# NuclearnAI/nuclear-sim

Measured on AMD Instinct MI355X. Metric: plant-env-steps/s, higher is better.
Workload: dtype f64

## Files before the change

nuclear_sim_amd/csrc/npd_step4.h:

```cpp
#ifndef NPD_STEP4_H
#define NPD_STEP4_H

#define NPD4_THREADS 256
#ifndef NPD4_NO_ELIDE
#define NPD4_ST_STORE(T, stype, s, old, inst) NPD_ST_STORE_ELIDE(T, stype, s, old, inst)
#else
#define NPD4_ST_STORE(T, stype, s, old, inst) NPD_ST_STORE(T, stype, s, inst)
#endif
#define NPD4_SLOTS 142
#ifdef NPB_STAMPS
#define NPD4_STAMP(k) do { if (lane == 0 && npb_stamp_buf) npb_stamp_buf[((size_t)blockIdx.x * 4 + wave) * 32 + (k)] = __builtin_readcyclecounter(); } while (0)
#else
#define NPD4_STAMP(k)
#endif
enum { FL_CHAIN = 0, FL_FWFLOW = 1, FL_PRIM = 2, FL_FWCTL = 3, FL_PUMP = 4 , FL_SG = 8 , FL_PASSA = 11, FL_UNIT = 12 ,
       FL_POST = 15 , FL_VERDICT = 18, FL_TAIL = 19, FL_CONDP = 20, FL_LUBE = 21, FL_CHAINDONE = 22, FL_COUNT = 23 };
#define NPD4_FLAGP(n) ((volatile int *)&xch[Y_FLAGS * NPB_WAVE + 2 * (n)])
#define NPD4_FLAG_SET(n, v) do { asm volatile("" ::: "memory"); *NPD4_FLAGP(n) = (v); asm volatile("" ::: "memory"); } while (0)
#ifndef NPD4_POLL_SLEEP
#define NPD4_POLL_SLEEP 1
#endif
#define NPD4_FLAG_WAIT(n, v) do { while (__builtin_amdgcn_readfirstlane(*NPD4_FLAGP(n)) < (v)) __builtin_amdgcn_s_sleep(NPD4_POLL_SLEEP); asm volatile("" ::: "memory"); } while (0)
#define NPD4_UNIT_WAIT(u) do { if ((u) < 12) NPD4_FLAG_WAIT(FL_UNIT + (u) % 2, (u) / 2 + 1); else NPD4_FLAG_WAIT(FL_UNIT + 2, (u) - 11); } while (0)

enum {
  Y_EXTF = 0, Y_TIN = 5, Y_STEAM = 6, Y_CHRES = 7,
  Y_CFLOW = 0, Y_CIN = 3, Y_COUT = 6, Y_LDF = 9, Y_FWTEMP = 10, Y_NPREV = 11, Y_FPP = 12, Y_MAXLVL = 13, Y_RUNCOUNT = 14, Y_FWFLOW = 15,
  Y_PRIM = 16,
  Y_TIME = 22, Y_FLAGS = 23, Y_MAINT_TAB = 24,
  Y_PUMP = 25,
  Y_SAT = 25, Y_HG = 40, Y_TRATIO = 55, Y_HGEXT = 69,
  Y_OBS = 25, Y_INFO = 48,
  Y_SG = 77,
  Y_TOUT = 77,
  Y_PSELF = 95, Y_PEXT = 109, Y_PIN = 114,
  Y_TAIL = 95,
  Y_LOADING = 116, Y_STRESS = 130, Y_CWT = 140, Y_CONDP = 141
};
static_assert(Y_PUMP + 4 * X_PUMP_N <= Y_SG && Y_HGEXT + 5 <= Y_SG && Y_INFO + NPB_OBS_PAD <= Y_SG && Y_OBS + NPB_OBS_PAD <= Y_INFO && Y_SG + 18 <= Y_PSELF &&
              Y_TOUT + 14 <= Y_PSELF && Y_TAIL + 21 <= Y_LOADING && Y_PIN < Y_LOADING && Y_LOADING + 14 <= Y_STRESS && Y_STRESS + 8 <= Y_CWT && Y_CHRES + 7 <= Y_FWFLOW &&
              Y_CONDP < NPD4_SLOTS && 2 * FL_COUNT <= NPB_WAVE && NPD_MH_N + 8 <= NPB_WAVE, "exchange slot plan");

template <int K0, int K1>
__device__ __forceinline__ void npd4_store_turb_range(const npd_stage_t &st, const npb_turb_t &t, const npb_turb_t &t_old) {
  const double *d = reinterpret_cast<const double *>(&t), *od = reinterpret_cast<const double *>(&t_old);
#pragma unroll
  for (int k = K0; k < K1; k++) {
    if ((NPD_ELIDE_TURB_F >> k) & 1) {
      if (__builtin_amdgcn_ballot_w64(npd_real_bits(d[k]) != npd_real_bits(od[k])) != 0) *NPD_RP(NPD_SEC_COL(TURB, 0) + k) = (npd_real_t)d[k];
    } else {
      *NPD_RP(NPD_SEC_COL(TURB, 0) + k) = (npd_real_t)d[k];
    }
  }
}

#ifndef NPD4_UNITS_FIRST
#define NPD4_UNITS_FIRST 1
#endif
template <int R>
__device__ __forceinline__ void npd4_stage_preload(const npd_stage_t &st, npd_tstg_old_t &old) {
#define NPD4_OLD(member, k) (old.v[NPD_TSTG_SLOT(member, k)] = (double)NPD2_TSTG(member, k))
#pragma unroll
  for (int j = 0; j < 5; j++) {
    const int k = R + 3 * j;
    if (k >= 14) continue;
    NPD4_OLD(stage_efficiency_degradation, k); NPD4_OLD(stage_deposit_thickness, k);
    NPD4_OLD(stage_blade_wear_factor, k); NPD4_OLD(blade_temperatures, k);
    if (k < 8) NPD4_OLD(rotor_temperatures, k);
    if (k < 6) NPD4_OLD(casing_temperatures, k);
  }
#undef NPD4_OLD
}
template <int R>
__device__ __forceinline__ void npd4_stage_post(const npd_stage_t &st, const npd_tstg_old_t &old, double *xch, int lane, double tdt) {
  NPD4_FLAG_WAIT(FL_VERDICT, 1);
  const int base = (__builtin_amdgcn_readfirstlane(*NPD4_FLAGP(FL_VERDICT)) == 2) ? 100 : 0;
#pragma unroll
  for (int j = 0; j < 5; j++) {
    const int k = R + 3 * j;
    if (k >= 14) continue;
    NPD4_FLAG_WAIT(FL_CHAIN, base + k + 1);
    const double stress = npd_stage_post<NPD_SM>(st, k, old, XR(Y_LOADING + k), XR(Y_TOUT + k), tdt).stress;
    if (k < 8) XW(Y_STRESS + (k < 8 ? k : 0), stress);
  }
  NPD4_FLAG_SET(FL_POST + R, 1);
}
template <int U0, int STEP, int COUNT, int WHOSE>
__device__ __forceinline__ void npd4_pass_b_units(double *xch, int lane) {
#pragma unroll
  for (int j = 0; j < COUNT; j++) {
    const int u = U0 + STEP * j;
    if (u == 0) {
      NPD4_FLAG_WAIT(FL_PASSA, 1);
      const double sat = npd_tsat_antoine(XR(Y_PIN));
      XW(Y_SAT + 0, sat); XW(Y_HG + 0, npd_hg_from_tsat(sat));
    } else {
      const int k = u - 1;
      NPD4_FLAG_WAIT(FL_PASSA, k + 2);
      const double pk = XR(Y_PSELF + (k >= 0 ? k : 0)), pkm = (k == 0) ? XR(Y_PIN) : XR(Y_PSELF + (k > 0 ? k - 1 : 0));
      const double sat = npd_tsat_antoine(pk);
      XW(Y_SAT + u, sat); XW(Y_HG + u, npd_hg_from_tsat(sat)); XW(Y_TRATIO + (k >= 0 ? k : 0), npd_sqrt(npd_sqrt(pk / pkm)));
      if (NPD_IS_EXT(k)) XW(Y_HGEXT + NPD_EXT_IDX(k), npd_hg_from_tsat(npd_tsat_antoine(XR(Y_PEXT + NPD_EXT_IDX(k)))));
    }
    NPD4_FLAG_SET(FL_UNIT + WHOSE, j + 1);
  }
}

#define NPD4_PUMP(i_, BEFORE_THE_STORE) \
  { \
    const int i = (i_); \
    npb_pump_t pm; \
    NPD_ST_LOAD(PUMP, npb_pump_t, pm, i);       \
    NPD4_FLAG_WAIT(FL_FWCTL, 1); \
    const int n_prev_running = (int)XR(Y_NPREV); \
    const double flow_per_pump = XR(Y_FPP); \
    npd_pump_sysconds_t sc; \
    sc.feedwater_temperature = 40.0; sc.suction_pressure = 0.5; sc.discharge_pressure = 7.4; sc.max_sg_level = XR(Y_MAXLVL); \
    const double maint_time = maint_clock; \
    if (maint) { asm volatile("s_waitcnt vmcnt(0)" ::: "memory"); npd_maint_cache_landed(maint_cache); } \
    const uint32_t cooling_mask = (i & 1) ? maint_cache.z : maint_cache.x; \
    const float cooling_until = __uint_as_float((i & 1) ? maint_cache.w : maint_cache.y); \
    const npb_pump_t pm_old = pm; \
    if (!serial_pumps) { \
      npd_fw_pump_update(&pm, 1, n_prev_running, flow_per_pump, &sc, dt);         \
    } else { \
      int running_count = 0; \
      if (i > 0) { NPD4_FLAG_WAIT(FL_PUMP + (i > 0 ? i - 1 : 0), 1); running_count = (int)XR(Y_RUNCOUNT); } \
      npd_fw_pump_update(&pm, running_count < n_prev_running, n_prev_running, flow_per_pump, &sc, dt); \
      XW(Y_RUNCOUNT, (double)(running_count + (pm.status == NPD_PUMP_RUNNING))); \
    } \
    npd2_publish_pump(xch + (Y_PUMP - X_PUMP) * NPB_WAVE, lane, i, pm); \
    NPD4_FLAG_SET(FL_PUMP + i, 1); \
    if (maint) {    \
      if (__builtin_amdgcn_ballot_w64(npd_maint_pump_hit(&pm, maint_tab, cooling_mask, cooling_until, maint_time)) != 0) maint_hit_bits |= 1u << i; \
    } \
    BEFORE_THE_STORE; \
    NPD4_ST_STORE(PUMP, npb_pump_t, pm, pm_old, i); \
  }

template <int WHO, bool MAINT>
__device__ __forceinline__ void npd_step4_body(
    const npb_params_t &P, int n_plants, size_t N, npd_real_t *__restrict__ f64,
    const int32_t *__restrict__ action, const double *__restrict__ magnitude, const double *__restrict__ setpoint,
    const double *__restrict__ noise_z, const double *__restrict__ cw_temp, double *__restrict__ obs_out,
    double *__restrict__ reward_out, uint8_t *__restrict__ done_out, uint32_t *__restrict__ trip_out,
    double *__restrict__ info_out, const npd_maint_hot_t &MH, const npd_maint_rule_consts_t *maint_rc, const npd_maint_cache_t &MC) {
  __shared__ __attribute__((aligned(16))) double xch[NPD4_SLOTS * NPB_WAVE];
  const int lane = threadIdx.x & (NPB_WAVE - 1);
  const int wave = __builtin_amdgcn_readfirstlane(threadIdx.x >> 6);
  const int my_pump = (wave == 3) ? 0 : (wave == 0 ? 3 : wave);
  const size_t block_base = (size_t)blockIdx.x * NPB_WAVE;
  if (block_base >= (size_t)n_plants) return;
  NPD_SEGMENT(f64, N, block_base);
  const size_t p = block_base + lane;
  const bool live = p < (size_t)n_plants;
  const double dt = P.dt, tdt = dt / 60.0;
  const bool kinetics = P.heat_source == NPB_HEAT_REACTOR;
  npd_stage_t st;
  {
    st.lds = (char *)xch;
    st.f64b = (npd_gchar_t *)(f64 + block_base);
    st.nr = (uint32_t)(N * NPD_RB);
    st.laner = (uint32_t)lane * NPD_RB;
    st.grp16 = 0;
    st.diag = nullptr; st.diag_pitch = 0;
  }
  const bool maint = MAINT && P.maint_enabled && maint_rc != nullptr;
  unsigned maint_hit_bits = 0, maint_due_with_orders = 0;
  double *const maint_tab = xch + Y_MAINT_TAB * NPB_WAVE;
  NPD4_STAMP(0);
  npd_u32x4 maint_cache = {0, 0, 0, 0};
  if (maint) maint_cache = npd_maint_cache_fetch(MC, p, my_pump >> 1);
  double maint_clock = 0.0;
  if (maint) maint_clock = (double)NPD_ST_F64(PRIM, npb_prim_t, sim_time, 0, 0);
  bool serial_pumps;
  {
    const int fw_mask = *NPD_NP(const int32_t, NPD_SEC_COL(FW, 0) + NPB_FW_NCARRY + (NPB_FW_NOUT + NPB_I32_SLOT(npb_fw_t, FW, running_mask)) / NPD_NPC,
                                (NPB_FW_NOUT + NPB_I32_SLOT(npb_fw_t, FW, running_mask)) % NPD_NPC);
    int n_prev = 0, may_run = 0;
#pragma unroll
    for (int i = 0; i < NPB_NUM_PUMPS; i++) {
      n_prev += (fw_mask >> i) & 1;
      const int stt = *NPD_NP(const int32_t, NPD_SEC_COL(PUMP, i) + NPB_PUMP_NCARRY + (NPB_PUMP_NOUT + NPB_I32_SLOT(npb_pump_t, PUMP, status)) / NPD_NPC,
                              (NPB_PUMP_NOUT + NPB_I32_SLOT(npb_pump_t, PUMP, status)) % NPD_NPC);
      may_run += (stt == NPD_PUMP_RUNNING || stt == NPD_PUMP_STARTING);
    }
    if (wave == 3 && lane < FL_COUNT) *NPD4_FLAGP(lane) = 0;
    serial_pumps = __builtin_amdgcn_ballot_w64(n_prev > 0 && may_run > n_prev) != 0;
    if (maint) { asm volatile("s_waitcnt vmcnt(0)" ::: "memory"); maint_clock += dt; }
  }
  NPD2_SYNC_();

  if (wave == 3) {
    npb_fw_t fw; npb_fw_t fw_old;
    double prev_levels[NPB_NUM_SG];
    double prev_feedwater_temp = 0.0, cw_old = 0.0, operating_hours = 0.0, cooling_water_temperature = 0.0, actual_feedwater_temp = 0.0;
    __builtin_amdgcn_s_setprio(3);
    double maint_entry = 0.0;
    if (maint && lane < NPD_MH_N) maint_entry = MH.tab[lane];
    cooling_water_temperature = (double)NPD_ST_F64(SEC, npb_sec_t, cooling_water_temperature, 0, 0);
    cw_old = cooling_water_temperature;
    prev_feedwater_temp = (double)NPD_ST_F64(SEC, npb_sec_t, previous_feedwater_temp, 0, 0);
    operating_hours = (double)NPD_ST_F64(SEC, npb_sec_t, operating_hours, 0, 0);
    const int has_prev = *NPD_NP(const int32_t, NPD_SEC_COL(SEC, 0) + NPB_SEC_NCARRY + (NPB_SEC_NOUT + NPB_I32_SLOT(npb_sec_t, SEC, has_previous_sg_conditions)) / NPD_NPC,
                                 (NPB_SEC_NOUT + NPB_I32_SLOT(npb_sec_t, SEC, has_previous_sg_conditions)) % NPD_NPC);
    double prev_flows[NPB_NUM_SG], prev_quals[NPB_NUM_SG];
#pragma unroll
    for (int i = 0; i < NPB_NUM_SG; i++) {
      prev_levels[i] = (double)NPD_ST_F64(SEC, npb_sec_t, prev_sg_levels, 0, i);
      prev_flows[i] = (double)NPD_ST_F64(SEC, npb_sec_t, prev_sg_steam_flows, 0, i);
      prev_quals[i] = (double)NPD_ST_F64(SEC, npb_sec_t, prev_sg_qualities, 0, i);
    }
    const double cw_in = (live && cw_temp) ? cw_temp[p] : NAN;
    if (!isnan(cw_in)) cooling_water_temperature = cw_in;
    actual_feedwater_temp = npd_feedwater_temp(prev_feedwater_temp);
    NPD_ST_LOAD(FW, npb_fw_t, fw, 0);
    fw_old = fw;
    if (__builtin_amdgcn_ballot_w64(!has_prev) != 0) {
      NPD4_FLAG_WAIT(FL_PRIM, 1);
      const double load_demand_fraction = XR(Y_LDF);
      if (!has_prev) npd_first_step_sg_conditions(load_demand_fraction, prev_levels, prev_flows, prev_quals);
    }
    const double total_flow_demand = npd_fw_level_control(&fw, prev_levels, prev_flows, prev_quals, dt);
    int n_prev_running = 0;
#pragma unroll
    for (int i = 0; i < NPB_NUM_PUMPS; i++) n_prev_running += (fw.running_mask >> i) & 1;
    const double flow_per_pump = (n_prev_running > 0) ? total_flow_demand / n_prev_running : 0.0;
    XW(Y_FWTEMP, actual_feedwater_temp); XW(Y_NPREV, (double)n_prev_running); XW(Y_FPP, flow_per_pump);
    XW(Y_MAXLVL, npd_pymax3(prev_levels[0], prev_levels[1], prev_levels[2]));
    if (maint && lane < NPD_MH_N) maint_tab[lane] = maint_entry;
    NPD4_FLAG_SET(FL_FWCTL, 1);
    __builtin_amdgcn_s_setprio(0);
    NPD4_STAMP(1);
    NPD4_PUMP(0, (void)0);
    NPD4_STAMP(2);
    NPD4_FLAG_WAIT(FL_PUMP + 1, 1); NPD4_FLAG_WAIT(FL_PUMP + 2, 1); NPD4_FLAG_WAIT(FL_PUMP + 3, 1);
    NPD4_STAMP(3);
    __builtin_amdgcn_s_setprio(3);
    npb_turb_t t; npb_turb_t t_old;
    double fw_total_flow = 0.0, fw_total_power = 0.0;
    int fw_available = 0; uint32_t trip_flags = 0;
    npd_fw_acc_t acc;
    acc.total_flow = acc.total_power = acc.flow_sum = 0.0;
    acc.total_cavitation_risk = acc.total_wear_level = acc.total_vibration = 0.0;
    acc.running_count = acc.running_mask = acc.trips = 0; acc.trip_mask = 0; acc.trip_kinds = 0;
#pragma unroll
    for (int i = 0; i < NPB_NUM_PUMPS; i++) npd_fw_pump_tail(npd_pump_vals_read(xch + (Y_PUMP + i * X_PUMP_N) * NPB_WAVE, lane), i, &fw, &acc, dt);
    npd_fw_result_t fwr;
    npd_fw_finish(&fw, &acc, prev_levels, dt, &fwr);
    fw_total_flow = fwr.total_flow_rate; fw_total_power = fwr.total_power_consumption;
    fw_available = fwr.system_availability;
    trip_flags = (fwr.pump_trip_mask << 8) | (fw.system_trip_active ? NPB_TRIP_FW_SYSTEM : 0);
    XW(Y_FWFLOW, fw_total_flow);
    NPD4_FLAG_SET(FL_FWFLOW, 1);
    __builtin_amdgcn_s_setprio(0);
    NPD4_STAMP(4);
    NPD_ST_LOAD(TURB, npb_turb_t, t, 0);
    NPD4_ST_STORE(FW, npb_fw_t, fw, fw_old, 0);
    t_old = t;
    npd_tstg_old_t old;
    npd4_stage_preload<2>(st, old);
    NPD4_STAMP(5);
    NPD4_FLAG_WAIT(FL_SG + 0, 1); NPD4_FLAG_WAIT(FL_SG + 1, 1); NPD4_FLAG_WAIT(FL_SG + 2, 1);
    NPD4_STAMP(6);
    __builtin_amdgcn_s_setprio(3);
    double sg_total_thermal = 0.0, sg_total_steam = 0.0, sg_avg_pressure = 0.0, sg_avg_temperature = 0.0, sg_avg_quality = 0.0;
    int sg_system_availability = 0;
    double pressure_stability_factor = 1.0, load_demand = 0.0;
    bool seq = false;
    double sg_ap = 0.0, sg_at = 0.0, sg_aq = 0.0, sg_pressures[NPB_NUM_SG];
    int sg_effective = 0;
#pragma unroll
    for (int i = 0; i < NPB_NUM_SG; i++) {
      const int b = Y_SG + 6 * i;
      sg_total_thermal += XR(b + 0); sg_total_steam += XR(b + 1);
      sg_ap += XR(b + 2); sg_at += XR(b + 3); sg_aq += XR(b + 4);
      sg_pressures[i] = XR(b + 2);
      if (XR(b + 5) != 0.0) sg_effective++;
    }
    sg_avg_pressure = sg_ap / NPB_NUM_SG; sg_avg_temperature = sg_at / NPB_NUM_SG; sg_avg_quality = sg_aq / NPB_NUM_SG;
    sg_system_availability = sg_effective >= (NPB_NUM_SG - 1);
    load_demand = XR(Y_PRIM + 1);
    t.load_demand = load_demand;
    pressure_stability_factor = npd_pressure_stability_factor(sg_pressures);
    XW(Y_CWT, cooling_water_temperature);
    XW(Y_PIN, sg_avg_pressure); XW(Y_TIN, sg_avg_temperature); XW(Y_STEAM, sg_total_steam);
    NPD4_FLAG_SET(FL_PASSA, 1);
    {
      const double inlet_pressure = sg_avg_pressure, inlet_flow = sg_total_steam;
      bool rare = !(inlet_pressure >= 0.001 && inlet_pressure <= 22.0);
      double cur_p = inlet_pressure, cur_flow = inlet_flow;
#pragma unroll
      for (int k = 0; k < 14; k++) {
        double d_in, d_out, design_flow; int has_extraction, is_lp;
        npd_stage_design(k, &d_in, &d_out, &design_flow, &has_extraction, &is_lp);
        double design_pressure_ratio = d_out / d_in;
        double extraction_demand = (k == 2) ? 25.0 * load_demand : (k == 3) ? 30.0 * load_demand : (k == 4) ? 20.0 * load_demand
                                 : (k == 8) ? 15.0 * load_demand : (k == 9) ? 10.0 * load_demand : 0.0;
        double outlet_pressure = npd_stage_requested_outlet(k, cur_p, inlet_flow);
        rare = rare || (outlet_pressure >= cur_p);
        double min_allowed, max_allowed;
        if (k == 13) { min_allowed = 0.002; max_allowed = 0.009; }
        else { min_allowed = cur_p * (design_pressure_ratio * 0.7); max_allowed = cur_p * (design_pressure_ratio * 1.3); }
        double self_out = (outlet_pressure < min_allowed) ? min_allowed : ((outlet_pressure > max_allowed) ? max_allowed : outlet_pressure);
        rare = rare || (self_out != outlet_pressure);
        double ef = 0.0, pe = cur_p;
        if (has_extraction && extraction_demand > 0) {
          ef = npd_clip(extraction_demand, 5.0, npd_pymin(50.0, cur_flow * 0.3));
          pe = cur_p * 0.7 + outlet_pressure * (1 - 0.7);
        }
        if (NPD_IS_EXT(k)) { XW(Y_EXTF + NPD_EXT_IDX(k), ef); XW(Y_PEXT + NPD_EXT_IDX(k), pe); }
        const double flow_out_k = cur_flow - ef;
        rare = rare || !(self_out >= 0.001 && self_out <= 22.0) || !(pe >= 0.001 && pe <= 22.0) || !(outlet_pressure >= 0.001);
        cur_p = self_out; cur_flow = flow_out_k;
        XW(Y_PSELF + k, self_out);
        NPD4_FLAG_SET(FL_PASSA, k + 2);
      }
      seq = __builtin_amdgcn_ballot_w64(rare) != 0;
      NPD4_FLAG_SET(FL_VERDICT, seq ? 2 : 1);
    }
    __builtin_amdgcn_s_setprio(0);
    NPD4_STAMP(7);
    npd4_pass_b_units<12, 1, 3, 2>(xch, lane);
    npd4_stage_post<2>(st, old, xch, lane, tdt);
    NPD4_STAMP(8);
    NPD4_FLAG_WAIT(FL_CHAINDONE, 1);
    __builtin_amdgcn_s_setprio(3);
    const double stage_power_mw = XR(Y_CHRES + 0) * pressure_stability_factor;
    const double turbine_efficiency = XR(Y_CHRES + 5), hp_power = XR(Y_CHRES + 3), lp_power = XR(Y_CHRES + 4);
    double max_bearing_metal = 0.0, total_displacement = 0.0;
    npd_turbine_rotor(&t, stage_power_mw, sg_avg_temperature, load_demand, tdt, &max_bearing_metal, &total_displacement);
    NPD4_STAMP(9);
    NPD4_FLAG_WAIT(FL_POST + 0, 1); NPD4_FLAG_WAIT(FL_POST + 1, 1);
    NPD4_STAMP(10);
    double max_stress = 0.0;
#pragma unroll
    for (int k = 0; k < 8; k++) max_stress = (k == 0) ? XR(Y_STRESS) : npd_pymax(max_stress, XR(Y_STRESS + k));
    npd_turbine_protect(&t, stage_power_mw, max_stress, max_bearing_metal, total_displacement, sg_system_availability, 0.007, tdt);
    const npd_power_t pw = npd_power_gates(t.total_power_output * 0.98, XR(Y_PRIM + 4), fw_total_flow, sg_total_steam, sg_avg_pressure);
    if (t.trip_active) trip_flags |= NPB_TRIP_TURBINE;
    XW(Y_TAIL + 0, pw.electrical_power); XW(Y_TAIL + 1, pw.thermal_efficiency); XW(Y_TAIL + 2, sg_avg_pressure); XW(Y_TAIL + 3, sg_total_steam);
    XW(Y_TAIL + 4, fw_total_flow); XW(Y_TAIL + 5, pw.heat_rejection); XW(Y_TAIL + 6, sg_total_thermal); XW(Y_TAIL + 7, sg_avg_temperature);
    XW(Y_TAIL + 8, sg_avg_quality); XW(Y_TAIL + 9, (double)(sg_system_availability | (fw_available << 1))); XW(Y_TAIL + 10, prev_feedwater_temp);
    XW(Y_TAIL + 11, cw_old); XW(Y_TAIL + 12, operating_hours); XW(Y_TAIL + 13, t.total_power_output); XW(Y_TAIL + 14, fw_total_power);
    XW(Y_TAIL + 15, turbine_efficiency); XW(Y_TAIL + 16, hp_power); XW(Y_TAIL + 17, lp_power); XW(Y_TAIL + 18, (double)trip_flags);
    XW(Y_TAIL + 19, actual_feedwater_temp); XW(Y_TAIL + 20, (double)fw_available);
    NPD4_FLAG_SET(FL_TAIL, 1);
    __builtin_amdgcn_s_setprio(0);
    NPD4_STAMP(11);
    {
      constexpr int L0 = NPB_F64_SLOT(npb_turb_t, lub_oil_temperature);
      static_assert(NPB_F64_SLOT(npb_turb_t, load_demand) + 1 == L0, "turbine section layout");
      NPD4_FLAG_WAIT(FL_LUBE, 1);
      npd4_store_turb_range<0, L0>(st, t, t_old);
      static_assert(NPB_TURB_NOUT == 4 && NPB_TURB_NI32 == 2, "turbine narrow layout");
      constexpr int NC = NPB_TURB_NCARRY;
      *NPD_NP(float, NPD_SEC_COL(TURB, 0) + NC + 0 / NPD_NPC, 0 % NPD_NPC) = (float)t.thermal_expansion;
      *NPD_NP(float, NPD_SEC_COL(TURB, 0) + NC + 1 / NPD_NPC, 1 % NPD_NPC) = (float)t.total_power_output;
      *NPD_NP(float, NPD_SEC_COL(TURB, 0) + NC + 2 / NPD_NPC, 2 % NPD_NPC) = (float)t.vibration_displacement;
      *NPD_NP(int32_t, NPD_SEC_COL(TURB, 0) + NC + 4 / NPD_NPC, 4 % NPD_NPC) = t.trip_active;
      *NPD_NP(int32_t, NPD_SEC_COL(TURB, 0) + NC + 5 / NPD_NPC, 5 % NPD_NPC) = t.trip_latched_mask;
    }
    NPD4_FLAG_WAIT(FL_CONDP, 1);
    NPD4_STAMP(12);
    if (info_out) {
      const double condenser_pressure = XR(Y_CONDP), electrical_power = XR(Y_TAIL + 0), thermal_efficiency = XR(Y_TAIL + 1);
      const double sg_avg_pressure_t = XR(Y_TAIL + 2), sg_total_steam_t = XR(Y_TAIL + 3), heat_rejection = XR(Y_TAIL + 5);
      double info[NPB_INFO_DIM];
      npd_info_primary(info, XR(Y_PRIM + 2), XR(Y_PRIM + 3), XR(Y_TIME));
      npd_info_secondary(info, electrical_power, thermal_efficiency, sg_total_steam_t, sg_avg_pressure_t, condenser_pressure, heat_rejection,
                         XR(Y_TAIL + 4), XR(Y_TAIL + 6), XR(Y_TAIL + 13), XR(Y_TAIL + 14), XR(Y_PRIM + 4), XR(Y_TAIL + 15),
                         XR(Y_TAIL + 16), XR(Y_TAIL + 17));
      npd2_store_rows<NPB_INFO_DIM>(info, info_out, xch + Y_INFO * NPB_WAVE, lane, block_base, (size_t)n_plants);
    }
    NPD4_STAMP(13);
  } else {
    int scram_bits = 0;
    if (wave == 1) {
      npb_chem_t ch0; npb_ph_t ph;
      NPD_ST_LOAD(CHEM, npb_chem_t, ch0, 0);
      NPD_ST_LOAD(PH, npb_ph_t, ph, 0);
      const npb_chem_t ch0_old = ch0; const npb_ph_t ph_old = ph;
      npd_chemistry_sidecar(&ch0, &ph, dt);
      NPD4_ST_STORE(CHEM, npb_chem_t, ch0, ch0_old, 0);
      NPD4_ST_STORE(PH, npb_ph_t, ph, ph_old, 0);
    }
    if (wave == 0) {
      npd_maint_due_t maint_due = {};
      if (maint) npd_maint_due_load(&maint_due, f64, N, p);
      const npd_inputs_t in = npd_step_inputs(live, p, action, magnitude, setpoint, noise_z, nullptr);
      npb_prim_t s;
      if (kinetics) {
        NPD_ST_LOAD(PRIM, npb_prim_t, s, 0);
      } else {
        double *d = reinterpret_cast<double *>(&s);
  #pragma unroll
        for (int k = 0; k < NPD_PRIM_KIN0; k++) d[k] = (double)*NPD_RP(NPD_SEC_COL(PRIM, 0) + k);
  #pragma unroll
        for (int k = NPD_PRIM_KIN0; k < NPB_PRIM_NCARRY; k++) d[k] = 0.0;
  #pragma unroll
        for (int j = 0; j < NPB_PRIM_NOUT; j++) d[NPB_PRIM_NCARRY + j] = (double)*NPD_NP(const float, NPD_SEC_COL(PRIM, 0) + NPB_PRIM_NCARRY + j / NPD_NPC, j % NPD_NPC);
        int32_t *q = reinterpret_cast<int32_t *>(d + NPB_PRIM_NF64);
  #pragma unroll
        for (int k = 0; k < NPB_PRIM_NI32; k++) q[k] = *NPD_NP(const int32_t, NPD_SEC_COL(PRIM, 0) + NPB_PRIM_NCARRY + (NPB_PRIM_NOUT + k) / NPD_NPC, (NPB_PRIM_NOUT + k) % NPD_NPC);
      }
      const npb_prim_t s_old = s;
      if (P.heat_source != NPB_HEAT_EXTERNAL && !isnan(in.power_setpoint)) s.hs_setpoint_percent = npd_clip(in.power_setpoint, 0.0, 150.0);
      double rho[NPB_INFO_NRHO];
      int nan_reset;
      const int scram_fired = npd_primary_update(&s, &P, &in, &nan_reset, rho);
      npd_store_reactivity_components(P, rho, info_out, n_plants, p);
      npd_coupling_t c;
      npd_primary_to_secondary(&s, &c);
      double primary_thermal_power = 0.0;
  #pragma unroll
      for (int i = 0; i < NPB_NUM_SG; i++) {
        XW(Y_CFLOW + i, c.flow[i]); XW(Y_CIN + i, c.inlet_temp[i]); XW(Y_COUT + i, c.outlet_temp[i]);
        primary_thermal_power += c.thermal_power[i];
      }
      XW(Y_LDF, npd_load_demand_fraction(primary_thermal_power));
      s.sim_time += dt;
      scram_bits = (s.scram_status != 0) | (scram_fired ? 2 : 0) | (nan_reset ? 4 : 0);
      XW(Y_PRIM + 0, npd_base_reward(s)); XW(Y_PRIM + 1, s.power_level);
      XW(Y_PRIM + 2, s.thermal_power_mw); XW(Y_PRIM + 3, s.total_reactivity_pcm); XW(Y_PRIM + 4, primary_thermal_power);
      XW(Y_PRIM + 5, (double)scram_bits); XW(Y_TIME, s.sim_time);
      NPD4_FLAG_SET(FL_PRIM, 1);
      s.has_heat_removal_factor = 1;
      NPD_ST_STORE_ELIDE_PRIM(s, s_old);
      if (maint) {
        const bool work = npd_maint_due_decide(&maint_due, s.sim_time, MH.tab[2 * NPB_MAINT_NPARAM + 1]);
        maint_due_with_orders = __builtin_amdgcn_ballot_w64(work) != 0 ? 1u : 0u;
      }
    }
    NPD4_STAMP(1);
    npb_sg_t g;
    NPD4_PUMP(my_pump, NPD_ST_LOAD(SG, npb_sg_t, g, wave));
    NPD4_STAMP(2);
    {
      const int i = wave;
      NPD4_FLAG_WAIT(FL_PRIM, 1);
      NPD4_STAMP(3);
      const double c_flow = XR(Y_CFLOW + i), c_in = XR(Y_CIN + i), c_out = XR(Y_COUT + i);
      const double load_demand_fraction = XR(Y_LDF), feedwater_temp = XR(Y_FWTEMP);
      double total_primary_flow = 0.0;
      total_primary_flow += XR(Y_CFLOW + 0); total_primary_flow += XR(Y_CFLOW + 1); total_primary_flow += XR(Y_CFLOW + 2);
      const double actual_total_steam_flow = P.sg_design_total_steam_flow * load_demand_fraction;
      const double demand = (total_primary_flow > 0) ? actual_total_steam_flow * (c_flow / total_primary_flow) : actual_total_steam_flow / NPB_NUM_SG;
      const npb_sg_t g_old = g;
      const double level_old = (double)NPD_ST_F64(SEC, npb_sec_t, prev_sg_levels, 0, i);
      const double heat_transfer = npd_sg_part1(&g, &P, c_in, c_out, c_flow, dt * 60);
      NPD4_STAMP(4);
      NPD4_FLAG_WAIT(FL_FWFLOW, 1);
      NPD4_STAMP(5);
      const double fw_flow = XR(Y_FWFLOW);
      npd_sg_result_t r;
      r.heat_transfer_rate = 0.0; r.steam_flow_rate = 0.0; r.thermal_efficiency = 0.0;
      npd_sg_part2(&g, &P, heat_transfer, demand, fw_flow / NPB_NUM_SG, feedwater_temp, dt * 60, &r);
      const int b = Y_SG + 6 * i;
      XW(b + 0, r.heat_transfer_rate); XW(b + 1, r.steam_flow_rate); XW(b + 2, g.secondary_pressure);
      XW(b + 3, g.secondary_temperature); XW(b + 4, g.steam_quality); XW(b + 5, r.thermal_efficiency > 0.1 ? 1.0 : 0.0);
      NPD4_ST_STORE(SG, npb_sg_t, g, g_old, i);
      NPD_ST_F64_ELIDE(SEC, npb_sec_t, prev_sg_levels, 0, i, g.water_level, level_old);
      NPD_ST_F64(SEC, npb_sec_t, prev_sg_steam_flows, 0, i) = (npd_real_t)r.steam_flow_rate;
      NPD_ST_F64(SEC, npb_sec_t, prev_sg_qualities, 0, i) = (npd_real_t)g.steam_quality;
      NPD4_FLAG_SET(FL_SG + i, 1);
    }
    NPD4_STAMP(6);
    npd_tstg_old_t old;
    npb_cond_t cd, cd_old; npb_chem_t chc, chc_old;
    if (wave == 1) {
      double stage_eff[14];
#pragma unroll
      for (int k = 0; k < 14; k++) {
        const double deposit = (double)NPD2_TSTG(stage_deposit_thickness, k), eff_deg = (double)NPD2_TSTG(stage_efficiency_degradation, k);
        stage_eff[k] = npd_stage_total_efficiency(deposit, (double)NPD2_TSTG(stage_blade_wear_factor, k), eff_deg);
      }
      NPD4_STAMP(7);
      __builtin_amdgcn_s_setprio(3);
      NPD4_FLAG_WAIT(FL_PASSA, 1);
      const double sg_avg_pressure = XR(Y_PIN), sg_avg_temperature = XR(Y_TIN), sg_total_steam = XR(Y_STEAM), load_demand = XR(Y_PRIM + 1);
      npd_chain_t ch;
      ch.T_in = sg_avg_temperature; ch.total_power = 0.0; ch.total_extraction = 0.0; ch.lp6_outlet_enthalpy = 0.0;
      ch.hp_power = 0.0; ch.lp_power = 0.0; ch.h_in0 = 0.0;
      double turbine_efficiency = 0.0;
      {
        NPD4_UNIT_WAIT(0);
        ch.sat_in = XR(Y_SAT + 0); ch.hg_in = XR(Y_HG + 0);
        double cur_flow = sg_total_steam;
#pragma unroll
        for (int k = 0; k < 14; k++) {
          NPD4_UNIT_WAIT(k + 1);
          const double p_in = (k == 0) ? sg_avg_pressure : XR(Y_PSELF + (k > 0 ? k - 1 : 0)), p_self_k = XR(Y_PSELF + k);
          const double sat_k = XR(Y_SAT + k + 1), hg_k = XR(Y_HG + k + 1), tr_k = XR(Y_TRATIO + k);
          const double ef = NPD_IS_EXT(k) ? XR(Y_EXTF + NPD_EXT_IDX(k)) : 0.0;
          const double hgx = NPD_IS_EXT(k) ? XR(Y_HGEXT + NPD_EXT_IDX(k)) : 0.0;
          const double flow_out_k = cur_flow - ef;
          cur_flow = flow_out_k;
          double T_out, loading;
          npd_stage_chain(k, ch, p_in, p_self_k, sat_k, hg_k, tr_k, flow_out_k, ef, hgx, stage_eff[k], &T_out, &loading);
          XW(Y_TOUT + k, T_out); XW(Y_LOADING + k, loading);
          NPD4_FLAG_SET(FL_CHAIN, k + 1);
        }
        turbine_efficiency = npd_stage_overall_efficiency(ch, XR(Y_PSELF + 13), sg_total_steam);
      }
      NPD4_FLAG_WAIT(FL_VERDICT, 1);
      if (__builtin_amdgcn_readfirstlane(*NPD4_FLAGP(FL_VERDICT)) == 2) {
        ch.T_in = sg_avg_temperature; ch.total_power = 0.0; ch.total_extraction = 0.0; ch.lp6_outlet_enthalpy = 0.0;
        ch.hp_power = 0.0; ch.lp_power = 0.0; ch.h_in0 = 0.0;
        turbine_efficiency = 0.0;
        double cur_p = sg_avg_pressure, cur_T = sg_avg_temperature, cur_flow = sg_total_steam;
#pragma unroll
        for (int k = 0; k < 14; k++) {
          double T_out, loading;
          npd_stage_seq(k, cur_p, cur_T, cur_flow, sg_total_steam, load_demand, stage_eff[k], ch, &T_out, &loading);
          XW(Y_TOUT + k, T_out); XW(Y_LOADING + k, loading);
          NPD4_FLAG_SET(FL_CHAIN, 100 + k + 1);
        }
        turbine_efficiency = npd_stage_overall_efficiency_seq(sg_avg_temperature, sg_avg_pressure, cur_T, cur_p, sg_total_steam);
      }
      XW(Y_CHRES + 0, ch.total_power); XW(Y_CHRES + 1, ch.total_extraction); XW(Y_CHRES + 2, ch.lp6_outlet_enthalpy);
      XW(Y_CHRES + 3, ch.hp_power); XW(Y_CHRES + 4, ch.lp_power); XW(Y_CHRES + 5, turbine_efficiency);
      XW(Y_CHRES + 6, sg_total_steam - ch.total_extraction);
      NPD4_FLAG_SET(FL_CHAINDONE, 1);
      __builtin_amdgcn_s_setprio(0);
      NPD4_STAMP(8);
    } else if (wave == 0) {
#if NPD4_UNITS_FIRST
      npd4_pass_b_units<0, 2, 6, 0>(xch, lane); NPD4_STAMP(7); npd4_stage_preload<0>(st, old); NPD4_STAMP(8); npd4_stage_post<0>(st, old, xch, lane, tdt);
#else
      npd4_stage_preload<0>(st, old); NPD4_STAMP(7); npd4_pass_b_units<0, 2, 6, 0>(xch, lane); NPD4_STAMP(8); npd4_stage_post<0>(st, old, xch, lane, tdt);
#endif
    } else {
      npd4_stage_preload<1>(st, old); NPD4_STAMP(7); npd4_pass_b_units<1, 2, 6, 1>(xch, lane); NPD4_STAMP(8);
      NPD_ST_LOAD(COND, npb_cond_t, cd, 0);
      NPD_ST_LOAD(CHEM, npb_chem_t, chc, 1);
      cd_old = cd; chc_old = chc;
      npd4_stage_post<1>(st, old, xch, lane, tdt);
    }
    NPD4_STAMP(9);
    if (wave == 0) {
      double obs[NPB_OBS_DIM];
      obs[0] = (double)NPD_ST_F64(PRIM, npb_prim_t, neutron_flux, 0, 0) / 1e12;
      obs[1] = (double)NPD_ST_F64(PRIM, npb_prim_t, fuel_temperature, 0, 0) / 1000;
      obs[2] = (double)NPD_ST_F64(PRIM, npb_prim_t, coolant_temperature, 0, 0) / 300;
      obs[3] = (double)NPD_ST_F64(PRIM, npb_prim_t, coolant_pressure, 0, 0) / 20;
      obs[4] = (double)NPD_ST_F64(PRIM, npb_prim_t, coolant_flow_rate, 0, 0) / 50000;
      obs[5] = (double)NPD_ST_F64(PRIM, npb_prim_t, steam_temperature, 0, 0) / 300;
      obs[6] = (double)NPD_ST_F64(PRIM, npb_prim_t, steam_pressure, 0, 0) / 10;
      obs[8] = (double)NPD_ST_F64(PRIM, npb_prim_t, control_rod_position, 0, 0) / 100;
      obs[9] = (double)NPD_ST_F64(PRIM, npb_prim_t, steam_valve_position, 0, 0) / 100;
      obs[11] = (double)(scram_bits & 1);
      asm volatile("s_waitcnt vmcnt(0)" ::: "memory");
      NPD4_FLAG_WAIT(FL_TAIL, 1);
      __builtin_amdgcn_s_setprio(2);
      NPD4_STAMP(10);
      const double ld = XR(Y_PRIM + 1), sg_total_steam_t = XR(Y_TAIL + 3), fw_flow_t = XR(Y_TAIL + 4);
      obs[10] = ld / 100;
      npd_obs_secondary(obs, sg_total_steam_t, XR(Y_TAIL + 0), XR(Y_TAIL + 1), sg_total_steam_t, ld, XR(Y_CWT), fw_flow_t, XR(Y_TAIL + 14), XR(Y_TAIL + 20));
      uint32_t flags = (uint32_t)XR(Y_TAIL + 18);
      if (scram_bits & 1) flags |= NPB_TRIP_SCRAM;
      if (scram_bits & 2) flags |= NPB_TRIP_SCRAM_FIRED;
      if (scram_bits & 4) flags |= NPB_TRIP_NAN_RESET;
      if (live) {
        if (done_out) __builtin_nontemporal_store((uint8_t)((scram_bits >> 1) & 1), &done_out[p]);
        if (trip_out) __builtin_nontemporal_store(flags, &trip_out[p]);
      }
      if (obs_out) npd2_store_rows<NPB_OBS_DIM>(obs, obs_out, xch + Y_OBS * NPB_WAVE, lane, block_base, (size_t)n_plants);
      NPD4_STAMP(11);
    } else if (wave == 1) {
      {
        npb_turb_t t;
        NPD_ST_LOAD(TURB, npb_turb_t, t, 0);
        const npb_turb_t t_old = t;
        asm volatile("s_waitcnt vmcnt(0)" ::: "memory");
        NPD4_FLAG_SET(FL_LUBE, 1);
        npd_turbine_lube(&t, tdt);
        constexpr int L0 = NPB_F64_SLOT(npb_turb_t, lub_oil_temperature), L1 = NPB_F64_SLOT(npb_turb_t, thermal_expansion);
        static_assert(L1 == NPB_TURB_NCARRY, "lub_* carried members close the section");
        npd4_store_turb_range<L0, L1>(st, t, t_old);
        *NPD_NP(float, NPD_SEC_COL(TURB, 0) + NPB_TURB_NCARRY + 3 / NPD_NPC, 3 % NPD_NPC) = (float)t.lub_effectiveness;
      }
      NPD4_STAMP(10);
      NPD4_STAMP(11);
      NPD4_FLAG_WAIT(FL_TAIL, 1); NPD4_FLAG_WAIT(FL_CONDP, 1);
      NPD4_STAMP(12);
      const double condenser_pressure = XR(Y_CONDP);
      const double base_reward = XR(Y_PRIM + 0), ld = XR(Y_PRIM + 1);
      const double electrical_power = XR(Y_TAIL + 0), thermal_efficiency = XR(Y_TAIL + 1), sg_avg_pressure_t = XR(Y_TAIL + 2), sg_total_steam_t = XR(Y_TAIL + 3);
      const double reward = npd_reward(base_reward, thermal_efficiency, ld, electrical_power, sg_avg_pressure_t, condenser_pressure);
      if (live && reward_out) __builtin_nontemporal_store(reward, &reward_out[p]);
      const int avail = (int)XR(Y_TAIL + 9);
      NPD_ST_F64_ELIDE(SEC, npb_sec_t, previous_feedwater_temp, 0, 0, XR(Y_TAIL + 19), XR(Y_TAIL + 10));
      NPD_ST_F64_ELIDE(SEC, npb_sec_t, cooling_water_temperature, 0, 0, XR(Y_CWT), XR(Y_TAIL + 11));
      NPD_ST_F64(SEC, npb_sec_t, operating_hours, 0, 0) = (npd_real_t)(XR(Y_TAIL + 12) + dt / 3600.0);
      const npb_sec_t so = npd_sec_outputs(electrical_power, thermal_efficiency, sg_total_steam_t, XR(Y_TAIL + 6), XR(Y_TAIL + 4), ld,
                                           sg_avg_pressure_t, XR(Y_TAIL + 7), XR(Y_TAIL + 8), avail & 1);
      NPD_ST_STORE_NARROW(SEC, npb_sec_t, so, 0);
      NPD_ST_F64(PRIM, npb_prim_t, steam_flow_rate, 0, 0) = (npd_real_t)sg_total_steam_t;
      NPD_ST_F64(PRIM, npb_prim_t, last_heat_removal_factor, 0, 0) = (npd_real_t)npd_heat_removal_factor(sg_total_steam_t, avail & 2);
      NPD4_STAMP(13);
    } else {
      NPD4_FLAG_WAIT(FL_CHAINDONE, 1);
      __builtin_amdgcn_s_setprio(2);
      const double effective_steam_flow = XR(Y_CHRES + 6), lp6_outlet_enthalpy = XR(Y_CHRES + 2), cwt = XR(Y_CWT);
      const double lp_exhaust_quality = npd_lp_exhaust_quality(0.007, lp6_outlet_enthalpy);
      npd_condenser_result_t cr;
      npd_condenser_update(&cd, &chc, 0.007, effective_steam_flow, lp_exhaust_quality, 45000.0, cwt, 1.2, 185.0, tdt, &cr);
      XW(Y_CONDP, cr.condenser_pressure);
      NPD4_FLAG_SET(FL_CONDP, 1);
      NPD4_ST_STORE(COND, npb_cond_t, cd, cd_old, 0);
      NPD4_ST_STORE(CHEM, npb_chem_t, chc, chc_old, 1);
      NPD4_STAMP(10);
      NPD4_STAMP(12);
    }
  }
  NPD4_STAMP(31);
  if (maint) {
    volatile unsigned *handover = (volatile unsigned *)(maint_tab + 48);
    if (wave != 0 && lane == 0) handover[2 * wave] = maint_hit_bits;
    asm volatile("s_waitcnt vmcnt(0) lgkmcnt(0)\n\ts_barrier" ::: "memory");
    if (wave == 0) {
      unsigned bits = maint_hit_bits;
#pragma unroll
      for (int w = 1; w < 4; w++) bits |= (unsigned)__builtin_amdgcn_readfirstlane((int)handover[2 * w]);
      if (bits | maint_due_with_orders) npd_maint_rule_for_wave<WHO>(maint_rc, MC, f64, N, p, bits, maint_due_with_orders);
    }
  }
}

__global__ __launch_bounds__(NPD4_THREADS) __attribute__((amdgpu_waves_per_eu(2, 2))) void npb_step4_kernel(NPD2_KERNEL_ARGS) { npd_step4_body<6, false>(NPD2_KERNEL_PASS); }
__global__ __launch_bounds__(NPD4_THREADS) __attribute__((amdgpu_waves_per_eu(2, 2))) void npb_step4_maint_kernel(NPD2_KERNEL_ARGS) { npd_step4_body<6, true>(NPD2_KERNEL_PASS); }

#endif
```

Measured before the change: 746.0 million.

## Issue per-wave state loads before preamble barrier and hand over turbine/level data via LDS

Each wave now issues its own section loads (FW, CHEM/PH, PRIM, PUMP) before the preamble barrier, and only wave 3 computes the serial-pump decision, which it broadcasts through a new LDS flag slot. Previously every wave did the pump-status global loads and waited at the barrier before starting its own loads. Wave 1 no longer reloads turbine state or waits on the FL_LUBE flag. Wave 3 instead writes rotor speed, bearing values, load demand and the previous SG levels into new exchange slots, and flag pointers are typed as LDS address space so the compiler emits LDS accesses. This enlarges the per-group LDS footprint and adds handover writes, which could reduce occupancy.

```diff
diff --git a/nuclear_sim_amd/csrc/npd_step4.h b/nuclear_sim_amd/csrc/npd_step4.h
--- a/nuclear_sim_amd/csrc/npd_step4.h
+++ b/nuclear_sim_amd/csrc/npd_step4.h
@@ -7,15 +7,31 @@
 #else
 #define NPD4_ST_STORE(T, stype, s, old, inst) NPD_ST_STORE(T, stype, s, inst)
 #endif
-#define NPD4_SLOTS 142
+#ifndef NPD4_EARLY_LOADS
+#define NPD4_EARLY_LOADS 1
+#endif
+#ifndef NPD4_LDS_HANDOVER
+#define NPD4_LDS_HANDOVER 1
+#endif
+#define NPD4_SLOTS (142 + 10 * NPD4_LDS_HANDOVER)
+static_assert(2 * NPD4_SLOTS * NPB_WAVE * 8 <= 160 * 1024, "two groups must fit a CU's LDS");
 #ifdef NPB_STAMPS
 #define NPD4_STAMP(k) do { if (lane == 0 && npb_stamp_buf) npb_stamp_buf[((size_t)blockIdx.x * 4 + wave) * 32 + (k)] = __builtin_readcyclecounter(); } while (0)
 #else
 #define NPD4_STAMP(k)
 #endif
 enum { FL_CHAIN = 0, FL_FWFLOW = 1, FL_PRIM = 2, FL_FWCTL = 3, FL_PUMP = 4 , FL_SG = 8 , FL_PASSA = 11, FL_UNIT = 12 ,
-       FL_POST = 15 , FL_VERDICT = 18, FL_TAIL = 19, FL_CONDP = 20, FL_LUBE = 21, FL_CHAINDONE = 22, FL_COUNT = 23 };
-#define NPD4_FLAGP(n) ((volatile int *)&xch[Y_FLAGS * NPB_WAVE + 2 * (n)])
+       FL_POST = 15 , FL_VERDICT = 18, FL_TAIL = 19, FL_CONDP = 20, FL_LUBE = 21, FL_CHAINDONE = 22, FL_COUNT = 23,
+       FL_SERIAL = 23  };
+#ifndef NPD4_LDS_FLAGS
+#define NPD4_LDS_FLAGS 1
+#endif
+#if NPD4_LDS_FLAGS
+typedef __attribute__((address_space(3))) volatile int npd4_flag_t;
+#else
+typedef volatile int npd4_flag_t;
+#endif
+#define NPD4_FLAGP(n) ((npd4_flag_t *)&xch[Y_FLAGS * NPB_WAVE + 2 * (n)])
 #define NPD4_FLAG_SET(n, v) do { asm volatile("" ::: "memory"); *NPD4_FLAGP(n) = (v); asm volatile("" ::: "memory"); } while (0)
 #ifndef NPD4_POLL_SLEEP
 #define NPD4_POLL_SLEEP 1
@@ -35,11 +51,14 @@
   Y_TOUT = 77,
   Y_PSELF = 95, Y_PEXT = 109, Y_PIN = 114,
   Y_TAIL = 95,
-  Y_LOADING = 116, Y_STRESS = 130, Y_CWT = 140, Y_CONDP = 141
+  Y_LOADING = 116, Y_STRESS = 130, Y_CWT = 140, Y_CONDP = 141,
+  Y_LUBE = 142,
+  Y_LEVELS = 142
 };
 static_assert(Y_PUMP + 4 * X_PUMP_N <= Y_SG && Y_HGEXT + 5 <= Y_SG && Y_INFO + NPB_OBS_PAD <= Y_SG && Y_OBS + NPB_OBS_PAD <= Y_INFO && Y_SG + 18 <= Y_PSELF &&
               Y_TOUT + 14 <= Y_PSELF && Y_TAIL + 21 <= Y_LOADING && Y_PIN < Y_LOADING && Y_LOADING + 14 <= Y_STRESS && Y_STRESS + 8 <= Y_CWT && Y_CHRES + 7 <= Y_FWFLOW &&
-              Y_CONDP < NPD4_SLOTS && 2 * FL_COUNT <= NPB_WAVE && NPD_MH_N + 8 <= NPB_WAVE, "exchange slot plan");
+              Y_CONDP < Y_LUBE && (!NPD4_LDS_HANDOVER || (Y_LUBE + 10 <= NPD4_SLOTS && Y_LEVELS + NPB_NUM_SG <= NPD4_SLOTS)) &&
+              2 * (FL_SERIAL + 1) <= NPB_WAVE && NPD_MH_N + 8 <= NPB_WAVE, "exchange slot plan");
 
 template <int K0, int K1>
 __device__ __forceinline__ void npd4_store_turb_range(const npd_stage_t &st, const npb_turb_t &t, const npb_turb_t &t_old) {
@@ -106,11 +125,11 @@
   }
 }
 
-#define NPD4_PUMP(i_, BEFORE_THE_STORE) \
+#define NPD4_PUMP(i_, THE_LOAD, BEFORE_THE_STORE) \
   { \
     const int i = (i_); \
     npb_pump_t pm; \
-    NPD_ST_LOAD(PUMP, npb_pump_t, pm, i);       \
+    THE_LOAD;                                   \
     NPD4_FLAG_WAIT(FL_FWCTL, 1); \
     const int n_prev_running = (int)XR(Y_NPREV); \
     const double flow_per_pump = XR(Y_FPP); \
@@ -173,23 +192,34 @@
   if (maint) maint_cache = npd_maint_cache_fetch(MC, p, my_pump >> 1);
   double maint_clock = 0.0;
   if (maint) maint_clock = (double)NPD_ST_F64(PRIM, npb_prim_t, sim_time, 0, 0);
-  bool serial_pumps;
-  {
-    const int fw_mask = *NPD_NP(const int32_t, NPD_SEC_COL(FW, 0) + NPB_FW_NCARRY + (NPB_FW_NOUT + NPB_I32_SLOT(npb_fw_t, FW, running_mask)) / NPD_NPC,
-                                (NPB_FW_NOUT + NPB_I32_SLOT(npb_fw_t, FW, running_mask)) % NPD_NPC);
-    int n_prev = 0, may_run = 0;
-#pragma unroll
-    for (int i = 0; i < NPB_NUM_PUMPS; i++) {
-      n_prev += (fw_mask >> i) & 1;
-      const int stt = *NPD_NP(const int32_t, NPD_SEC_COL(PUMP, i) + NPB_PUMP_NCARRY + (NPB_PUMP_NOUT + NPB_I32_SLOT(npb_pump_t, PUMP, status)) / NPD_NPC,
-                              (NPB_PUMP_NOUT + NPB_I32_SLOT(npb_pump_t, PUMP, status)) % NPD_NPC);
-      may_run += (stt == NPD_PUMP_RUNNING || stt == NPD_PUMP_STARTING);
-    }
-    if (wave == 3 && lane < FL_COUNT) *NPD4_FLAGP(lane) = 0;
-    serial_pumps = __builtin_amdgcn_ballot_w64(n_prev > 0 && may_run > n_prev) != 0;
-    if (maint) { asm volatile("s_waitcnt vmcnt(0)" ::: "memory"); maint_clock += dt; }
-  }
-  NPD2_SYNC_();
+  bool serial_pumps = false;
+  if (wave == 3 && lane < FL_COUNT) *NPD4_FLAGP(lane) = 0;
+  int fw_mask = 0, pump_status[NPB_NUM_PUMPS] = {};
+  if (!NPD4_EARLY_LOADS || wave == 3) {
+    fw_mask = *NPD_NP(const int32_t, NPD_SEC_COL(FW, 0) + NPB_FW_NCARRY + (NPB_FW_NOUT + NPB_I32_SLOT(npb_fw_t, FW, running_mask)) / NPD_NPC,
+                      (NPB_FW_NOUT + NPB_I32_SLOT(npb_fw_t, FW, running_mask)) % NPD_NPC);
+#pragma unroll
+    for (int i = 0; i < NPB_NUM_PUMPS; i++)
+      pump_status[i] = *NPD_NP(const int32_t, NPD_SEC_COL(PUMP, i) + NPB_PUMP_NCARRY + (NPB_PUMP_NOUT + NPB_I32_SLOT(npb_pump_t, PUMP, status)) / NPD_NPC,
+                               (NPB_PUMP_NOUT + NPB_I32_SLOT(npb_pump_t, PUMP, status)) % NPD_NPC);
+  }
+#define NPD4_PREAMBLE_SYNC() do { \
+    if (!NPD4_EARLY_LOADS || wave == 3) { \
+      int n_prev = 0, may_run = 0; \
+      _Pragma("unroll") for (int i = 0; i < NPB_NUM_PUMPS; i++) { \
+        n_prev += (fw_mask >> i) & 1; \
+        may_run += (pump_status[i] == NPD_PUMP_RUNNING || pump_status[i] == NPD_PUMP_STARTING); \
+      } \
+      serial_pumps = __builtin_amdgcn_ballot_w64(n_prev > 0 && may_run > n_prev) != 0; \
+      if (NPD4_EARLY_LOADS && lane == 0) *NPD4_FLAGP(FL_SERIAL) = serial_pumps; \
+    } \
+    if (maint) { asm volatile("s_waitcnt vmcnt(0)" ::: "memory"); maint_clock += dt; } \
+    NPD2_SYNC_(); \
+    if (NPD4_EARLY_LOADS && wave != 3) serial_pumps = __builtin_amdgcn_readfirstlane(*NPD4_FLAGP(FL_SERIAL)) != 0; \
+  } while (0)
+#if !NPD4_EARLY_LOADS
+  NPD4_PREAMBLE_SYNC();
+#endif
 
   if (wave == 3) {
     npb_fw_t fw; npb_fw_t fw_old;
@@ -199,7 +229,6 @@
     double maint_entry = 0.0;
     if (maint && lane < NPD_MH_N) maint_entry = MH.tab[lane];
     cooling_water_temperature = (double)NPD_ST_F64(SEC, npb_sec_t, cooling_water_temperature, 0, 0);
-    cw_old = cooling_water_temperature;
     prev_feedwater_temp = (double)NPD_ST_F64(SEC, npb_sec_t, previous_feedwater_temp, 0, 0);
     operating_hours = (double)NPD_ST_F64(SEC, npb_sec_t, operating_hours, 0, 0);
     const int has_prev = *NPD_NP(const int32_t, NPD_SEC_COL(SEC, 0) + NPB_SEC_NCARRY + (NPB_SEC_NOUT + NPB_I32_SLOT(npb_sec_t, SEC, has_previous_sg_conditions)) / NPD_NPC,
@@ -212,10 +241,18 @@
       prev_quals[i] = (double)NPD_ST_F64(SEC, npb_sec_t, prev_sg_qualities, 0, i);
     }
     const double cw_in = (live && cw_temp) ? cw_temp[p] : NAN;
+    NPD_ST_LOAD(FW, npb_fw_t, fw, 0);
+#if NPD4_EARLY_LOADS
+    NPD4_PREAMBLE_SYNC();
+#endif
+    cw_old = cooling_water_temperature;
     if (!isnan(cw_in)) cooling_water_temperature = cw_in;
     actual_feedwater_temp = npd_feedwater_temp(prev_feedwater_temp);
-    NPD_ST_LOAD(FW, npb_fw_t, fw, 0);
     fw_old = fw;
+#if NPD4_LDS_HANDOVER
+#pragma unroll
+    for (int i = 0; i < NPB_NUM_SG; i++) XW(Y_LEVELS + i, prev_levels[i]);
+#endif
     if (__builtin_amdgcn_ballot_w64(!has_prev) != 0) {
       NPD4_FLAG_WAIT(FL_PRIM, 1);
       const double load_demand_fraction = XR(Y_LDF);
@@ -232,7 +269,7 @@
     NPD4_FLAG_SET(FL_FWCTL, 1);
     __builtin_amdgcn_s_setprio(0);
     NPD4_STAMP(1);
-    NPD4_PUMP(0, (void)0);
+    NPD4_PUMP(0, NPD_ST_LOAD(PUMP, npb_pump_t, pm, i), (void)0);
     NPD4_STAMP(2);
     NPD4_FLAG_WAIT(FL_PUMP + 1, 1); NPD4_FLAG_WAIT(FL_PUMP + 2, 1); NPD4_FLAG_WAIT(FL_PUMP + 3, 1);
     NPD4_STAMP(3);
@@ -285,6 +322,11 @@
     pressure_stability_factor = npd_pressure_stability_factor(sg_pressures);
     XW(Y_CWT, cooling_water_temperature);
     XW(Y_PIN, sg_avg_pressure); XW(Y_TIN, sg_avg_temperature); XW(Y_STEAM, sg_total_steam);
+#if NPD4_LDS_HANDOVER
+    XW(Y_LUBE + 0, t_old.rotor_speed); XW(Y_LUBE + 9, t_old.load_demand);
+#pragma unroll
+    for (int i = 0; i < 4; i++) { XW(Y_LUBE + 1 + i, t_old.bearing_load[i]); XW(Y_LUBE + 5 + i, t_old.bearing_metal_temp[i]); }
+#endif
     NPD4_FLAG_SET(FL_PASSA, 1);
     {
       const double inlet_pressure = sg_avg_pressure, inlet_flow = sg_total_steam;
@@ -351,7 +393,9 @@
     {
       constexpr int L0 = NPB_F64_SLOT(npb_turb_t, lub_oil_temperature);
       static_assert(NPB_F64_SLOT(npb_turb_t, load_demand) + 1 == L0, "turbine section layout");
+#if !NPD4_LDS_HANDOVER
       NPD4_FLAG_WAIT(FL_LUBE, 1);
+#endif
       npd4_store_turb_range<0, L0>(st, t, t_old);
       static_assert(NPB_TURB_NOUT == 4 && NPB_TURB_NI32 == 2, "turbine narrow layout");
       constexpr int NC = NPB_TURB_NCARRY;
@@ -378,8 +422,11 @@
     int scram_bits = 0;
     if (wave == 1) {
       npb_chem_t ch0; npb_ph_t ph;
+      NPD_ST_LOAD(PH, npb_ph_t, ph, 0);
       NPD_ST_LOAD(CHEM, npb_chem_t, ch0, 0);
-      NPD_ST_LOAD(PH, npb_ph_t, ph, 0);
+#if NPD4_EARLY_LOADS
+      NPD4_PREAMBLE_SYNC();
+#endif
       const npb_chem_t ch0_old = ch0; const npb_ph_t ph_old = ph;
       npd_chemistry_sidecar(&ch0, &ph, dt);
       NPD4_ST_STORE(CHEM, npb_chem_t, ch0, ch0_old, 0);
@@ -404,6 +451,9 @@
   #pragma unroll
         for (int k = 0; k < NPB_PRIM_NI32; k++) q[k] = *NPD_NP(const int32_t, NPD_SEC_COL(PRIM, 0) + NPB_PRIM_NCARRY + (NPB_PRIM_NOUT + k) / NPD_NPC, (NPB_PRIM_NOUT + k) % NPD_NPC);
       }
+#if NPD4_EARLY_LOADS
+      NPD4_PREAMBLE_SYNC();
+#endif
       const npb_prim_t s_old = s;
       if (P.heat_source != NPB_HEAT_EXTERNAL && !isnan(in.power_setpoint)) s.hs_setpoint_percent = npd_clip(in.power_setpoint, 0.0, 150.0);
       double rho[NPB_INFO_NRHO];
@@ -432,9 +482,20 @@
         maint_due_with_orders = __builtin_amdgcn_ballot_w64(work) != 0 ? 1u : 0u;
       }
     }
+#if NPD4_EARLY_LOADS
+    npb_pump_t pm2;
+    if (wave == 2) {
+      NPD_ST_LOAD(PUMP, npb_pump_t, pm2, my_pump);
+      NPD4_PREAMBLE_SYNC();
+    }
+#define NPD4_PUMP_LOAD if (wave == 2) pm = pm2; else NPD_ST_LOAD(PUMP, npb_pump_t, pm, i)
+#else
+#define NPD4_PUMP_LOAD NPD_ST_LOAD(PUMP, npb_pump_t, pm, i)
+#endif
     NPD4_STAMP(1);
     npb_sg_t g;
-    NPD4_PUMP(my_pump, NPD_ST_LOAD(SG, npb_sg_t, g, wave));
+    NPD4_PUMP(my_pump, NPD4_PUMP_LOAD, NPD_ST_LOAD(SG, npb_sg_t, g, wave));
+#undef NPD4_PUMP_LOAD
     NPD4_STAMP(2);
     {
       const int i = wave;
@@ -447,7 +508,11 @@
       const double actual_total_steam_flow = P.sg_design_total_steam_flow * load_demand_fraction;
       const double demand = (total_primary_flow > 0) ? actual_total_steam_flow * (c_flow / total_primary_flow) : actual_total_steam_flow / NPB_NUM_SG;
       const npb_sg_t g_old = g;
+#if NPD4_LDS_HANDOVER
+      const double level_old = XR(Y_LEVELS + i);
+#else
       const double level_old = (double)NPD_ST_F64(SEC, npb_sec_t, prev_sg_levels, 0, i);
+#endif
       const double heat_transfer = npd_sg_part1(&g, &P, c_in, c_out, c_flow, dt * 60);
       NPD4_STAMP(4);
       NPD4_FLAG_WAIT(FL_FWFLOW, 1);
@@ -569,14 +634,27 @@
       NPD4_STAMP(11);
     } else if (wave == 1) {
       {
-        npb_turb_t t;
+        npb_turb_t t = {};
+        constexpr int L0 = NPB_F64_SLOT(npb_turb_t, lub_oil_temperature), L1 = NPB_F64_SLOT(npb_turb_t, thermal_expansion);
+        static_assert(L1 == NPB_TURB_NCARRY, "lub_* carried members close the section");
+#if NPD4_LDS_HANDOVER
+        {
+          double *d = reinterpret_cast<double *>(&t);
+#pragma unroll
+          for (int k = L0; k < L1; k++) d[k] = (double)*NPD_RP(NPD_SEC_COL(TURB, 0) + k);
+          t.lub_effectiveness = (double)*NPD_NP(const float, NPD_SEC_COL(TURB, 0) + NPB_TURB_NCARRY + 3 / NPD_NPC, 3 % NPD_NPC);
+          t.rotor_speed = XR(Y_LUBE + 0); t.load_demand = XR(Y_LUBE + 9);
+#pragma unroll
+          for (int i = 0; i < 4; i++) { t.bearing_load[i] = XR(Y_LUBE + 1 + i); t.bearing_metal_temp[i] = XR(Y_LUBE + 5 + i); }
+        }
+        const npb_turb_t t_old = t;
+#else
         NPD_ST_LOAD(TURB, npb_turb_t, t, 0);
         const npb_turb_t t_old = t;
         asm volatile("s_waitcnt vmcnt(0)" ::: "memory");
         NPD4_FLAG_SET(FL_LUBE, 1);
+#endif
         npd_turbine_lube(&t, tdt);
-        constexpr int L0 = NPB_F64_SLOT(npb_turb_t, lub_oil_temperature), L1 = NPB_F64_SLOT(npb_turb_t, thermal_expansion);
-        static_assert(L1 == NPB_TURB_NCARRY, "lub_* carried members close the section");
         npd4_store_turb_range<L0, L1>(st, t, t_old);
         *NPD_NP(float, NPD_SEC_COL(TURB, 0) + NPB_TURB_NCARRY + 3 / NPD_NPC, 3 % NPD_NPC) = (float)t.lub_effectiveness;
       }
```

New measurement: 770.3 million (median of 5 runs). 3.3% higher.
